# maiziezhoulab/FocalSV

Measured on AMD Instinct MI355X. Metric: target regions/sec (50 kb, 30x HiFi), higher is better.
Workload: dtype u32; 1 GPU; 256 synthetic 50 kb regions per GPU, 30x HiFi-like reads U(10k,20k), 0.2% error, seed 1000+i (BASELINE.json configs[1]); regions_per_gpu=256

## Files before the change

### focalsv_amd/csrc/asm.hip

```cpp
#include "asm_kernels.h"
#include "k_kmer.h"
#include "layout.h"
#include <algorithm>
#include <chrono>
#include <cstdio>
#include <cstdlib>
#include <cstring>
#include <vector>
#include <thread>
#include <atomic>

namespace {

enum { KN_SKETCH, KN_UNIQ, KN_CHAIN, KN_BPM, KN_RESCUE, KN_PATH_FAST, KN_PATH_DP, KN_CONSENSUS, KN_REPACK, KN_EXACT, KN_STITCH, KN_PARTITION, KN_BND, KN_BND_CONS,
       KN_UNIQ_LONG, KN_CHAIN_SPILL,
       KN_COUNT,
       ST_SKETCH = KN_COUNT, ST_CHAIN, ST_VERIFY, ST_PATH, ST_CONSENSUS, ST_FINAL };
const char *const kn_names[KN_COUNT] = {"k_sketch", "k_uniq", "k_chain", "k5_bpm", "k_rescue_accept", "k_path_fast", "k_path_dp", "k_consensus",
                                        "k_repack", "k_exact", "k_stitch", "k_partition", "k_bnd_tasks", "k_bnd_consensus", "k_uniq_long", "k_chain_spill"};
static_assert(KN_COUNT <= FSV_MAX_KERNEL_STATS, "fsv_asm_stats holds every kernel's row");
enum { PASS_NONE = -1, PASS_WINDOWS, PASS_JUNCTIONS, PASS_BCIG, PASS_COUNT };

struct KTimes {
    struct Rec { int k; hipEvent_t a, b; uint64_t bytes; };
// ... 74 lines not shown
    Dev<uint32_t> set_hits;
    Dev<int32_t> len, new_len, idx2, bc_idx;
    Dev<int32_t> bc_win;
    Dev<fsv_mz> mz; Dev<fsv_ovl> ovl, ovl_prev; Dev<fsv_hit> hits, hits_packed; Dev<fsv_piece> pieces; Dev<BndPatch> bnd_patch;
    Dev<fsv_wtask> tasks, tasks2, tasks3; Dev<fsv_wres> res, res2, res3; Dev<fsv_wpath> paths, paths2;
    Dev<uint4> cols_sb, ovl_c, upair_tab, upair_tab_sw, gwin_tab, bc_rec; Dev<uint2> site_rec; Dev<int8_t> site_vec;
    Dev<uint4> uq_ws, spill_list; Dev<uint8_t> spill_slab;
    Dev<uint64_t> cols;
    Dev<unsigned long long> tmp;
    Dev<uint8_t> cov3, bnd_bytes, exact_flag, cwin, thr_tab; Dev<uint16_t> cwin_len; Dev<char> contig_out, contig_all;
    KmerTableState km;
    FilterState fs;
    ChargeState ch;
    std::vector<uint32_t> h_store;
    int occ_sb = 0, occ_fr[3] = {0, 0, 0}, occ_wide = 0;
    ChainArgs last_chain;
    std::vector<uint32_t> h_word_off;
    std::vector<int32_t> h_len;
    const uint32_t *cur_store = nullptr;
    uint32_t n_reads = 0;
    fsv_asm_stats stats;
    uint64_t n_long_reads = 0, n_spilled_pairs = 0;
    KTimes kt;
    void *h_pin = nullptr; size_t h_pin_cap = 0;
    uint32_t *ct_of(int row) { return counters.p + (size_t)row * CT_SLOT; }
    size_t held() const
    {
        return cap_sum(store[0], store[1], cols_sb, contig_all, word_off, len, set_start, read_set, pair_base, mz, mz_off, mz_cnt, ovl, tasks, res, paths,
                       counters, dp_list, dp_list2, dp_list3, dp_list16, dp_list_e3, dp_wide, dp_xwide, cols_wide, set_cols, site_cnt, site_rec, site_off, site_vec,
                       site_cursor, redo, site_lists, read_dirty, cov3, lb, sr_store, brel_off, tasks2, res2, paths2, idx2, bc_idx, bc_rec, bc_win, left_list, fix_list,
// ... 778 lines not shown
    SL.bc_win = W.bc_win.p;
    return FSV_OK;
}

static int consensus_stage(fsv_ctx *ctx, AsmWs &W, Round &R)
{
    const fsv_asm_params &P = R.P; const Batch &B = R.B;
    const uint32_t n_gwin = R.n_gwin;
    TRY(consensus_setup(ctx, W, R));
    const ConsArgs &C = R.C;
    const bool partition = B.n_pairs && P.partition;
    SiteArgs SA{};
    SiteLists SL{};
    if (partition) TRY(partition_setup(ctx, W, R, SA, SL));
    if (partition && P.junction_cigars) TRY(junction_cigars(ctx, W, R, SA, SL));
    const dim3 grid_w((n_gwin + 7u) & ~7u);
    W.kt.begin(ctx, PASS_WINDOWS, KN_CONSENSUS, (uint64_t)n_gwin * (96 + 448));
    if (R.wide_bands) {
        if (partition) FSV_LAUNCH(ctx, ctx->stream, (k_consensus<FSV_EV_CAP_WIDE, 1>), grid_w, dim3(64), 0, C, n_gwin, SL);
        else FSV_LAUNCH(ctx, ctx->stream, (k_consensus<FSV_EV_CAP_WIDE, 0>), grid_w, dim3(64), 0, C, n_gwin, SL);
    } else {
        if (partition) FSV_LAUNCH(ctx, ctx->stream, (k_consensus<FSV_EV_CAP, 1>), grid_w, dim3(64), 0, C, n_gwin, SL);
        else FSV_LAUNCH(ctx, ctx->stream, (k_consensus<FSV_EV_CAP, 0>), grid_w, dim3(64), 0, C, n_gwin, SL);
    }
    W.kt.end(ctx);
    if (partition) {
        const uint32_t grid_l = std::min<uint32_t>(std::max(1u, n_gwin), (uint32_t)ctx->n_cu * 16);
        W.kt.begin(ctx, KN_PARTITION, (uint64_t)B.n_reads * 4);
        FSV_LAUNCH(ctx, ctx->stream, k_snp_sites, dim3(grid_l), dim3(64), 0, C, SA, SL);
        FSV_LAUNCH(ctx, ctx->stream, k_hap_partition, dim3(B.n_reads), dim3(64), 0, C, SA, W.ovl.p, W.ovl_c.p, SL);
// ... 1086 lines not shown
```

### focalsv_amd/csrc/k_consensus.h

```cpp
#pragma once

namespace {

struct ConsArgs {
    const uint32_t *store;
    const uint32_t *word_off;
    const int32_t *read_len;
    const uint32_t *read_set;
    const uint32_t *set_start;
    const uint32_t *pair_base;
    const uint32_t *gwin_off;
    const uint32_t *gwin_read;
    const uint4 *ovl_c;
    const uint4 *gwin_tab;
    const fsv_wtask *tasks;
    const fsv_wpath *paths;
    uint8_t *cwin;
    uint16_t *cwin_len;
    uint32_t *warn;
    uint32_t *changed;
    uint32_t n_reads;
    const uint32_t *read_dirty;
    uint8_t *cov3;
    int junction_vote;
// ... 196 lines not shown
        while (cur >= 0 && cur != S && L < FSV_DG_N) {
            int mx = 0, nx = -1;
            if (L < FSV_INS_MAXLEN + 4) rb[L] = D.base[cur];
            L++;
            for (int i = 0; i < D.in_n[cur]; i++) { const int e = D.in_e[cur][i]; if (D.e_alive[e]) { const int o = D.e_from[e], w = dg_weight(D, o, false); if (w > mx) { mx = w; nx = o; } } }
            cur = nx;
        }
        const int Lc = min(L, FSV_INS_MAXLEN + 4);
        for (int i = 0; i < Lc && i < FSV_INS_MAXLEN; i++) { const uint8_t b = rb[Lc - 1 - i]; seq |= (uint32_t)(b == 'A' ? 0u : b == 'C' ? 1u : b == 'G' ? 2u : 3u) << (2 * i); }
    }
    if (L > FSV_INS_MAXLEN) L = FSV_INS_MAXLEN;
    out_key = ((uint32_t)L << 24) | seq;
    return ws >= we ? ws : we;
}

__device__ __forceinline__ bool poa_decide(const int W[4], const int Ifl[4], int dl, int ni, int mi, uint32_t ikey, int own, bool homo, uint8_t *out)
{
    uint8_t nb = 0;
    bool kept = true;
    for (int visit = 0; visit < 2; visit++) {
        int maxc = -1, type = 0, edge = own, total = 0;
#pragma unroll
        for (int k = 0; k < 4; k++) {
            const int b = k == 0 ? own : (k - 1 < own ? k - 1 : k);
            if (W[b] == 0) continue;
            const int cw = ni ? W[b] - Ifl[b] : W[b];
            total += cw;
            if (cw > maxc) { maxc = cw; type = 0; edge = b; }
        }
        if (ni) { total += ni; if (mi > maxc) { maxc = mi; type = 1; } }
        if (dl) { total += dl; if (dl > maxc) { maxc = dl; type = 2; } }
        if (maxc * 5 >= total * 3 || (homo && maxc * 1000 >= total * 515)) {
            if (type == 1) { const int L = (int)(ikey >> 24); for (int b = 0; b < L; b++) out[1 + nb++] = (uint8_t)((ikey >> (2 * b)) & 3u); ni = 0; continue; }
            if (type == 2) { kept = false; break; }
            out[1 + nb++] = (uint8_t)edge;
            break;
        }
        out[1 + nb++] = (uint8_t)own;
        break;
    }
    out[0] = nb;
    return kept;
}

__device__ __forceinline__ void most_frequent_insertion(const uint32_t *s_evkey, const uint16_t *s_evnext, uint32_t head, int &mi, uint32_t &key)
{
    int bc = 0; uint32_t bk = 0;
    for (uint32_t i = head; i != 0xffffu; i = s_evnext[i]) {
        const uint32_t k1 = s_evkey[i];
        int cn = 0;
        for (uint32_t j2 = head; j2 != 0xffffu; j2 = s_evnext[j2]) cn += (s_evkey[j2] == k1);
        if (cn > bc || (cn == bc && k1 < bk)) { bc = cn; bk = k1; }
    }
    mi = bc; key = bk;
}

#define FSV_INSLIST 128
#define COV_LO(v) ((int)(int16_t)((v) & 0xffff))
#define COV_HI(v) (((int)(v) - COV_LO(v)) >> 16)

template <class F>
__device__ __forceinline__ bool homo_strict(F B, int site, int len)
{
    const int beg = max(0, site - 3), end = min(len - 1, site + 3);
    const uint32_t own = B(site);
    uint32_t f_ch = 4u, b_ch = 4u;
// ... 17 lines not shown
    for (int off = 1; off < 64; off <<= 1) { const int o = __shfl_up(v, off, 64); if (lane >= off) v += o; }
    return v;
}
__device__ __forceinline__ void load_path_ops(const fsv_wpath *P, uint2 (&pv)[13])
{
    const uint2 *src = reinterpret_cast<const uint2 *>(P->ops);
#pragma unroll
    for (int i = 0; i < 13; i++) pv[i] = src[i];
}
__device__ __forceinline__ void lane_columns(int lane, int n, int &c0, int &c1)
{
    const int per = (n + 63) / 64;
    c0 = min(n, lane * per); c1 = min(n, c0 + per);
}

struct TallyCols {
    uint32_t cnt[FSV_WINDOW + 1][3];
    int32_t cov[FSV_WINDOW + 2];
    uint32_t path[64][27];
    uint32_t xraw[28];
    uint32_t cover;

    __device__ __forceinline__ void reset(int lane)
    {
        for (int i = lane; i < (FSV_WINDOW + 1) * 3; i += 64) (&cnt[0][0])[i] = 0;
        for (int i = lane; i < FSV_WINDOW + 2; i += 64) cov[i] = 0;
        if (lane == 0) cover = 0;
    }
    __device__ __forceinline__ void stage_backbone(int lane, const uint32_t *__restrict__ x, int org, int len)
    {
        if (lane < 28) { const int wi = (org >> 4) - 1 + lane; xraw[lane] = (wi >= 0 && wi <= ((len + 15) >> 4)) ? x[wi] : 0u; }
    }
    __device__ __forceinline__ uint32_t xb(int org, int p) const { return (xraw[(p >> 4) - ((org >> 4) - 1)] >> ((p & 15) << 1)) & 3u; }
    __device__ __forceinline__ void cnt_add(int c, uint32_t b) { atomicAdd(&cnt[c][b >> 1], 1u << ((b & 1u) << 4)); }
    __device__ __forceinline__ uint32_t cnt_get(int c, uint32_t b) const { return (cnt[c][b >> 1] >> ((b & 1u) << 4)) & 0xffffu; }
    __device__ __forceinline__ uint32_t stage_path(int lane, const uint2 (&pv)[13])
    {
        uint32_t nz = 0;
#pragma unroll
        for (int i = 0; i < 13; i++) {
            path[lane][2 * i] = pv[i].x; path[lane][2 * i + 1] = pv[i].y;
            nz |= (pv[i].x ? 1u << (2 * i) : 0u) | (pv[i].y ? 2u << (2 * i) : 0u);
        }
        return nz;
    }
};

__device__ __forceinline__ bool split_sub_site(const int oa[4], int occ2, int arrived, int &alt)
{
    const int occ1 = oa[0] + oa[1] + oa[2] + oa[3];
    if (occ1 <= 1) return false;
    const int occ0 = arrived - occ1 - occ2;
    int mx = occ2;
    alt = -1;
#pragma unroll
    for (int b = 0; b < 4; b++) if (oa[b] > mx) { mx = oa[b]; alt = b; }
    if (occ0 == 0 || alt < 0 || mx <= 1) return false;
#pragma unroll
    for (int b = 0; b < 4; b++) if (oa[b] == mx && b != alt) return false;
    return (double)(occ0 + 1 + mx) / (double)(arrived + 1) >= 0.95 && (double)mx / (double)(arrived + 1 - (occ0 + 1)) >= 0.70;
}

template <int EVC>
struct Tally : TallyCols {
    uint32_t evkey[EVC];
    uint32_t evhead[FSV_WINDOW + 1];
    uint32_t fl[FSV_WINDOW + 1];
    uint32_t evn, nins, ndev;
    uint16_t evnext[EVC];
    uint16_t inslist[FSV_INSLIST];
    uint16_t devlist[FSV_WINDOW + 1];
    static_assert(sizeof(DagLds) <= sizeof(uint32_t) * 64 * 27 && (FSV_WINDOW + 1) * 14 <= sizeof(uint32_t) * 64 * 27,
                  "the DAG scratch and the decided columns live in the path buffer between the tally and the write-out");

    __device__ __forceinline__ DagLds &dag() { return *reinterpret_cast<DagLds *>(&path[0][0]); }
    __device__ __forceinline__ uint8_t (*out())[14] { return reinterpret_cast<uint8_t (*)[14]>(&path[0][0]); }

    __device__ __forceinline__ void reset(int lane)
    {
        TallyCols::reset(lane);
        for (int i = lane; i < FSV_WINDOW + 1; i += 64) evhead[i] = 0xffffu;
        for (int i = lane; i < FSV_WINDOW + 1; i += 64) fl[i] = 0;
        if (lane == 0) { evn = 0; nins = 0; ndev = 0; }
    }
    __device__ __forceinline__ void add_event(int c, uint32_t key)
    {
        const uint32_t ev = atomicAdd(&evn, 1u);
        if (ev < (uint32_t)EVC) { evkey[ev] = key; evnext[ev] = (uint16_t)atomicExch(&evhead[c], ev); }
    }

    __device__ __forceinline__ void answer_insertions(int n_cols)
    {
        DagLds &D = dag();
        const int n_list = (int)nins, n = n_list > FSV_INSLIST ? n_cols : n_list;
        for (int li = 0; li < n; li++) {
            const int c = n_list > FSV_INSLIST ? li : (int)inslist[li];
            const uint32_t head = evhead[c] & 0xffffu;
            if (head == 0xffffu || (evhead[c] & 0x10000u)) continue;
            int nk = 0;
            for (uint32_t i = head; i != 0xffffu; i = evnext[i]) { if (nk < FSV_DG_K) D.keys[nk] = evkey[i]; nk++; }
            uint32_t key = 0;
            int mi = dag_insertion(D, nk, key);
            if (mi < 0) most_frequent_insertion(evkey, evnext, head, mi, key);
            evkey[head] = key; evnext[head] = (uint16_t)mi;
            evhead[c] |= 0x10000u;
        }
    }

    template <class F>
    __device__ __forceinline__ bool decide_columns(int lane, int c0, int c1, int org, int n_cols, int len, bool verbatim, int ins_dag, F extra)
    {
        int run = 0, frun = 0;
        for (int c = c0; c < c1; c++) {
            const int v = cov[c];
            run += COV_LO(v); frun += COV_HI(v);
            if (cnt_get(c, 5u)) {
                const uint32_t head = evhead[c];
                bool same = true;
                if (head != 0xffffu) { const uint32_t k0 = evkey[head]; for (uint32_t i = evnext[head]; i != 0xffffu; i = evnext[i]) if (evkey[i] != k0) { same = false; break; } }
                if (!same && ins_dag) { const uint32_t k = atomicAdd(&nins, 1u); if (k < FSV_INSLIST) inslist[k] = (uint16_t)c; }
            }
        }
        int arrived = wave_incl_sum(run, lane) - run, farrived = wave_incl_sum(frun, lane) - frun;
        __syncthreads();
        if (lane == 0 && nins) answer_insertions(n_cols);
        __syncthreads();
        uint8_t (*o)[14] = out();
        for (int c = c0; c < c1; c++) {
            arrived += COV_LO(cov[c]);
            farrived += COV_HI(cov[c]);
            o[c][0] = 1; o[c][1] = (uint8_t)xb(org, org + c);
            if (!verbatim && (cnt[c][0] | cnt[c][1] | cnt[c][2]) != 0u) {
                cov[c] = (int32_t)(((uint32_t)arrived & 0xffffu) | ((uint32_t)farrived << 16));
                devlist[atomicAdd(&ndev, 1u)] = (uint16_t)c;
            }
        }
        __syncthreads();
        bool differs = false;
        for (uint32_t e = lane; e < ndev; e += 64) {
            const int c = (int)devlist[e];
            arrived = (int)(int16_t)((uint32_t)cov[c] & 0xffffu); farrived = (int)(int16_t)((uint32_t)cov[c] >> 16);
            const uint32_t own = xb(org, org + c);
            const bool homo = c > 0 && homo_strict([&](int pp) { return xb(org, pp); }, org + c - 1, len);
            int W[4], Ifl[4], dev = 0;
#pragma unroll
            for (int b = 0; b < 4; b++) { W[b] = (int)cnt_get(c, (uint32_t)b); dev += W[b]; Ifl[b] = (int)((fl[c] >> (b << 3)) & 0xffu); }
            const int dl = (int)cnt_get(c, 4u), ni = (int)cnt_get(c, 5u);
#pragma unroll
            for (int b = 0; b < 4; b++) if ((int)own == b) { W[b] += arrived - dev - dl + 1; Ifl[b] = farrived; }
            int mi = 0; uint32_t ikey = 0;
            if (ni) {
                const uint32_t hv = evhead[c], head = hv & 0xffffu;
                if (head != 0xffffu) {
                    ikey = evkey[head];
                    if (hv & 0x10000u) mi = (int)evnext[head];
                    else if (ins_dag) { for (uint32_t i = head; i != 0xffffu; i = evnext[i]) mi++; }
                    else most_frequent_insertion(evkey, evnext, head, mi, ikey);
                }
            }
            const bool kept = poa_decide(W, Ifl, dl, ni, mi, ikey, (int)own, homo, &o[c][0]);
            extra(c, arrived, kept);
            if (o[c][0] != 1 || o[c][1] != (uint8_t)own) differs = true;
        }
        __syncthreads();
        return differs;
    }
};

#define FSV_PEND_N 4
template <int EVC>
__device__ __forceinline__ void cons_flush(Tally<EVC> &S, const uint32_t *__restrict__ store, uint32_t y_word, int y_len, int y_rev, int ry_start,
                                           const uint32_t (&ent)[FSV_PEND_N], int n)
{
    uint32_t bits[FSV_PEND_N];
#pragma unroll
    for (int i = 0; i < FSV_PEND_N; i++) if (i < n) bits[i] = fetch16(store, y_word, y_len, y_rev, ry_start + (int)((ent[i] >> 9) & 1023u)).bits;
#pragma unroll
// ... 63 lines not shown
    return n2;
}

struct SiteLists {
    uint32_t *site_cnt;
    uint32_t *win_list;
    uint32_t *redo_list;
    uint32_t *win_n;
    const int32_t *bc_win;
};
template <int EVC, int MODE>
__device__ __forceinline__ void consensus_window(const ConsArgs &A, const uint32_t gw, const SiteLists &L)
{
    __shared__ Tally<EVC> S;
    __shared__ uint32_t s_anydev;
    const int lane = threadIdx.x;
    const uint4 gt = A.gwin_tab[gw];
    const uint32_t r = gt.x, pbase = gt.y, n_ovl = gt.z;
    const int g = (int)gt.w;
    const int xlen = A.read_len[r];
    const int gs = g * FSV_WINDOW, glen = min(FSV_WINDOW, xlen - gs);
    S.stage_backbone(lane, A.store + A.word_off[r], gs, xlen);
    uint8_t *dst = A.cwin + (size_t)gw * FSV_CW_STRIDE;
    if (A.read_dirty && !A.read_dirty[r]) {
        __syncthreads();
        for (int c = lane; c < glen; c += 64) dst[c] = (uint8_t)S.xb(gs, gs + c);
        if (lane == 0) { A.cwin_len[gw] = (uint16_t)glen; if (MODE == 1) L.site_cnt[gw] = 0u; }
        return;
    }
    S.reset(lane);
    if (lane == 0) s_anydev = 0;
    __syncthreads();
    for (uint32_t oi = lane; oi < n_ovl; oi += 64) {
        const uint4 oc = A.ovl_c[pbase + oi];
        const int o_x_s = (int)oc.x, o_n_win = (int)(oc.z & 0x7fffffffu);
        const int j = g - o_x_s / FSV_WINDOW;
        if (!(oc.z >> 31) || j < 0 || j >= o_n_win) continue;
        const uint32_t ti = oc.y + (uint32_t)j;
        const fsv_wpath *P = A.paths + ti;
        const uint4 h0 = *reinterpret_cast<const uint4 *>(P);
        const uint2 h1 = *reinterpret_cast<const uint2 *>((const uint8_t *)P + 16);
        uint2 pv[13];
        load_path_ops(P, pv);
        atomicAdd(&S.cover, 1u);
        if ((h0.w & 0xffu) != 1u) continue;
        const bool clean_path = (int16_t)(h0.z >> 16) == 0;
        const uint32_t nz = clean_path ? 0u : S.stage_path(lane, pv);
        const int ry_start = (int)h0.x, plen = (int)(int16_t)(h0.z & 0xffffu);
        const uint32_t y_word = h1.x; const int y_len = (int)h1.y, y_rev = (int)((h0.w >> 8) & 0xffu);
        const int xs = max(gs, o_x_s) - gs;
        bool pend = false;
        if (j > 0 && A.junction_vote) {
            const uint4 hp = *reinterpret_cast<const uint4 *>(A.paths + ti - 1);
            if ((hp.w & 0xffu) == 1u) {
                const int gap = ry_start - (int)hp.y - 1;
                if (gap > 0 && xs == 0) {
                    pend = true;
                    if (gap <= FSV_INS_MAXLEN) {
                        uint32_t key = (uint32_t)gap << 24;
                        for (int b = 0; b < gap; b++) key |= fsv_base_at(A.store, y_word, y_len, y_rev, ry_start - gap + b) << (2 * b);
                        S.add_event(0, key);
                    }
                }
            }
        }
        if (pend || nz) s_anydev = 1u;
        int n2 = 0;
        if (clean_path) { if (pend) S.cnt_add(xs, 5u); }
        else n2 = cons_walk<EVC>(S, S.path[lane], nz, plen, xs, glen, pend, A.store, y_word, y_len, y_rev, ry_start);
        atomicAdd(&S.cov[xs], 1);
        atomicAdd(&S.cov[xs + plen - n2], -1);
    }
    __syncthreads();
    const bool verbatim = S.cover < 3u || s_anydev == 0u;
    if (A.cov3 && lane == 0) A.cov3[gw] = S.cover >= 3u ? 1 : 0;
    if (S.evn > (uint32_t)EVC && lane == 0) atomicOr(&A.warn[r], (uint32_t)FSV_W_INS_EVENTS);
    const int bc_lo = (MODE == 1 && L.bc_win) ? L.bc_win[3 * (size_t)gw + 1] : 1, bc_hi = (MODE == 1 && L.bc_win) ? L.bc_win[3 * (size_t)gw + 2] : 0;
    bool site = false;
    int c0, c1;
    lane_columns(lane, glen, c0, c1);
    const bool differs = S.decide_columns(lane, c0, c1, gs, glen, xlen, verbatim, A.ins_dag, [&](int c, int arrived, bool) {
        if (MODE != 1) return;
        int oa[4], alt;
#pragma unroll
        for (int b = 0; b < 4; b++) oa[b] = (int)S.cnt_get(c, (uint32_t)b);
        if (oa[0] + oa[1] + oa[2] + oa[3] > 1 && c >= bc_lo && c <= bc_hi) site = true;
        if (split_sub_site(oa, (int)S.cnt_get(c, 4u), arrived, alt)) site = true;
    });
    if (differs && A.changed) A.changed[r] = 1u;
    if (MODE == 1) {
        const bool any_site = __ballot(site) != 0ull || (L.bc_win && L.bc_win[3 * (size_t)gw]);
        if (lane == 0) {
            L.site_cnt[gw] = any_site ? FSV_SITE_MARK : 0u;
            if (any_site) L.win_list[atomicAdd(&L.win_n[0], 1u)] = gw;
        }
    }
    uint8_t (*s_out)[14] = S.out();
    uint32_t mine = 0;
    for (int c = c0; c < c1; c++) mine += s_out[c][0];
    const int incl = wave_incl_sum((int)mine, lane);
    uint32_t off = (uint32_t)incl - mine;
    const uint32_t tot = (uint32_t)__shfl(incl, 63, 64);
    if (tot > FSV_CW_STRIDE) {
        for (int c = lane; c < glen; c += 64) dst[c] = (uint8_t)S.xb(gs, gs + c);
        if (lane == 0) { A.cwin_len[gw] = (uint16_t)glen; atomicOr(&A.warn[r], (uint32_t)FSV_W_WINDOW_KEPT); }
        return;
    }
    for (int c = c0; c < c1; c++) for (int b = 0; b < s_out[c][0]; b++) dst[off++] = s_out[c][1 + b];
    if (lane == 0) A.cwin_len[gw] = (uint16_t)tot;
}

template <int EVC, int MODE>
__global__ __launch_bounds__(64) void k_consensus(ConsArgs A, uint32_t n_gwin, SiteLists L)
{
    uint32_t gw;
    if (xcd_block(n_gwin, gw)) consensus_window<EVC, MODE>(A, gw, L);
}

template <int EVC>
__global__ __launch_bounds__(64) void k_consensus_redo(ConsArgs A, SiteLists L)
{
    const uint32_t n = L.win_n[1];
    for (uint32_t i = blockIdx.x; i < n; i += gridDim.x) {
// ... 175 lines not shown
    uint32_t *site_cnt;
    uint2 *site_rec;
    uint32_t *site_off;
    uint32_t *rec_cursor; uint32_t rec_cap;
    int8_t *vec;
    uint32_t *vec_cursor;
    uint32_t vec_cap;
    uint32_t *read_sites;
    const int32_t *bc_idx;
    const uint4 *bc_rec;
    const fsv_wpath *bc_paths;
};

__device__ __forceinline__ void snp_sites_window(const ConsArgs &A, const uint32_t gw, const SiteArgs &S)
{
    __shared__ TallyCols T;
    __shared__ uint8_t s_alt[FSV_WINDOW + 1];
    __shared__ uint8_t s_sidx[FSV_WINDOW + 1];
    __shared__ uint32_t s_nsite, s_vbase, s_rbase;
    __shared__ uint32_t s_scan[64];
    const int lane = threadIdx.x;
    const uint4 gt = A.gwin_tab[gw];
    const uint32_t r = gt.x, pbase = gt.y, n_ovl = gt.z;
    const int g = (int)gt.w;
    const int xlen = A.read_len[r];
    const int gs = g * FSV_WINDOW, glen = min(FSV_WINDOW, xlen - gs);
    if (lane == 0) S.site_cnt[gw] = 0;
    T.stage_backbone(lane, A.store + A.word_off[r], gs, xlen);
    T.reset(lane);
    for (int i = lane; i < FSV_WINDOW + 1; i += 64) s_alt[i] = 0;
    if (lane == 0) s_nsite = 0;
// ... 378 lines not shown
                                                     const uint32_t *__restrict__ n3)
{
    const uint32_t j = blockIdx.x * blockDim.x + threadIdx.x;
    if (j < *n3) res2[src3[j]] = res3[j];
}

struct BndPatch { uint16_t ts, told, tnew, hs, hold, hnew, valid, pad; };

template <int EVC>
__global__ __launch_bounds__(64) void k_bnd_consensus(ConsArgs A, BndArgs B, const fsv_wpath *__restrict__ paths2, const uint32_t *__restrict__ store2,
                                                      BndPatch *__restrict__ patch, uint8_t *__restrict__ patch_bytes)
{
    static_assert(2 * FSV_BND_HALF + 1 <= FSV_WINDOW, "a junction's backbone fits the tally of a window");
    struct Lds : Tally<EVC> {
        uint32_t terr;
        uint16_t off[FSV_WINDOW + 2];
        uint8_t own[FSV_WINDOW + 1];
    };
    __shared__ Lds S;
    const int lane = threadIdx.x;
    const uint32_t n_list = *B.n_bnd;
    for (uint32_t li = blockIdx.x; li < n_list; li += gridDim.x) {
        __syncthreads();
        const uint32_t gw = B.bnd_list[li];
        const uint4 gt = A.gwin_tab[gw];
        const uint32_t r = gt.x, pbase = gt.y, n_ovl = gt.z;
        const int g = (int)gt.w;
        const int gs = g * FSV_WINDOW;
        const int LB = (int)B.lb[gw], len_now = LB + (int)B.cwin_len[gw];
        const int cws = max(0, LB - FSV_BND_HALF), cwe = min(len_now - 1, LB + FSV_BND_HALF - 1), blen = cwe - cws + 1;
        if (lane == 0) { patch[gw].valid = 0; S.terr = 0; }
        S.stage_backbone(lane, store2 + B.b_base + B.brel_off[r], cws, len_now);
        S.reset(lane);
        __syncthreads();
        for (uint32_t oi = lane; oi < n_ovl; oi += 64) {
            const uint4 oc = A.ovl_c[pbase + oi];
            const int o_x_s = (int)oc.x, o_n_win = (int)(oc.z & 0x7fffffffu);
            const int j = g - o_x_s / FSV_WINDOW;
            if (!(oc.z >> 31) || j < 0 || j >= o_n_win || o_x_s > gs) continue;
            const int32_t slot = B.idx2[oc.y + (uint32_t)j];
            if (slot == -2) { atomicAdd(&S.cover, 1u); atomicAdd(&S.cov[0], 1); atomicAdd(&S.cov[blen], -1); continue; }
            if (slot < 0) continue;
            const fsv_wpath *P = paths2 + slot;
            const uint4 h0 = *reinterpret_cast<const uint4 *>(P);
            if ((h0.w & 0xffu) != 1u) continue;
            const uint2 h1 = *reinterpret_cast<const uint2 *>((const uint8_t *)P + 16);
            const int perr = (int)(int16_t)(h0.z >> 16);
            atomicAdd(&S.cover, 1u);
            const int ry_start = (int)h0.x, plen = (int)(int16_t)(h0.z & 0xffffu);
            int n2 = 0;
            if (perr != 0) {
                atomicAdd(&S.terr, (uint32_t)perr);
                uint2 pv[13];
                load_path_ops(P, pv);
                const uint32_t nz = S.stage_path(lane, pv);
                n2 = cons_walk<EVC>(S, S.path[lane], nz, plen, 0, blen, false, A.store, h1.x, (int)h1.y, (int)((h0.w >> 8) & 0xffu), ry_start);
            }
            atomicAdd(&S.cov[0], 1);
            atomicAdd(&S.cov[plen - n2], -1);
        }
        __syncthreads();
        if (S.cover < 3u || S.terr == 0u) continue;
        if (S.evn > (uint32_t)EVC && lane == 0) atomicOr(&A.warn[r], (uint32_t)FSV_W_INS_EVENTS);
        int c0, c1;
        lane_columns(lane, blen, c0, c1);
        for (int c = c0; c < c1; c++) S.own[c] = 1;
        const bool differs = S.decide_columns(lane, c0, c1, cws, blen, len_now, false, A.ins_dag, [&](int c, int, bool kept) { S.own[c] = kept; });
        uint8_t (*s_out)[14] = S.out();
        int mine = 0;
        for (int c = c0; c < c1; c++) mine += s_out[c][0];
        if (__ballot(differs) == 0ull) continue;
        int off = wave_incl_sum(mine, lane) - mine;
        for (int c = c0; c < c1; c++) { S.off[c] = (uint16_t)off; off += s_out[c][0]; }
        const int sb = FSV_BND_SIDE, eb = blen - 1 - FSV_BND_SIDE;
        int fs = 0x7fffffff, fe = 0x7fffffff;
        for (int c = c0; c < c1; c++) { if (S.own[c] && c >= sb && c < fs) fs = c; if (S.own[c] && c >= eb && c < fe) fe = c; }
        for (int d = 32; d >= 1; d >>= 1) { fs = min(fs, __shfl_xor(fs, d)); fe = min(fe, __shfl_xor(fe, d)); }
        __syncthreads();
        if (eb <= sb || fs == 0x7fffffff || fe == 0x7fffffff) continue;
        const int o0 = (int)S.off[fs] + s_out[fs][0] - 1, o1 = (int)S.off[fe] + s_out[fe][0] - 1;
        const int R0 = cws + fs, R1 = cws + fe, sc = LB - cws;
        const int o_split = sc <= fs ? o0 : (sc > fe ? o1 + 1 : (int)S.off[sc]);
        const int lb_prev = (int)B.lb[gw - 1];
        BndPatch bp;
        bp.valid = 1; bp.pad = 0;
        bp.ts = (uint16_t)max(0, R0 - lb_prev); bp.told = (uint16_t)max(0, min(R1, LB - 1) - R0 + 1); bp.tnew = (uint16_t)(o_split - o0);
        bp.hs = (uint16_t)(max(R0, LB) - LB); bp.hold = (uint16_t)max(0, R1 - max(R0, LB) + 1); bp.hnew = (uint16_t)(o1 + 1 - o_split);
        if (R0 < lb_prev || o1 + 1 - o0 > FSV_CW_STRIDE) {
            if (lane == 0) atomicOr(&A.warn[r], (uint32_t)FSV_W_WINDOW_KEPT);
            continue;
        }
        uint8_t *dst = patch_bytes + (size_t)gw * FSV_CW_STRIDE;
        for (int c = c0; c < c1; c++)
            for (int b = 0; b < s_out[c][0]; b++) { const int pos = (int)S.off[c] + b; if (pos >= o0 && pos <= o1) dst[pos - o0] = s_out[c][1 + b]; }
        if (lane == 0) patch[gw] = bp;
    }
}

__global__ __launch_bounds__(64) void k_bnd_apply(const uint32_t *__restrict__ gwin_read, const uint32_t *__restrict__ gwin_off, const BndPatch *__restrict__ patch,
                                                  const uint8_t *__restrict__ patch_bytes, const uint32_t *__restrict__ bnd_flag, uint32_t n_gwin,
                                                  uint8_t *__restrict__ cwin, uint16_t *__restrict__ cwin_len, uint32_t *__restrict__ changed, uint32_t *__restrict__ warn)
{
    __shared__ uint8_t s_old[FSV_CW_STRIDE];
    const uint32_t gw = blockIdx.x;
    if (gw >= n_gwin) return;
    const uint32_t r = gwin_read[gw];
    const bool has_h = gw > gwin_off[r] && (bnd_flag[gw] & 1u) && patch[gw].valid;
    const bool has_t = gw + 1 < gwin_off[r + 1] && (bnd_flag[gw + 1] & 1u) && patch[gw + 1].valid;
    if (!has_h && !has_t) return;
// ... 30 lines not shown
```

Measured before the change: 2529 regions/s.

## Shrink consensus LDS footprint to fit more windows per CU

Cuts the consensus and junction-consensus tally shared memory. The per-lane path staging shrinks from 64 rows to 31 rows, processed in ballot-ranked batches. Decided columns are packed into one byte each, with insertion bases re-read from the event key at write-out, and event heads become 16-bit packed words updated by CAS. The goal is to raise resident blocks per CU (a static_assert targets 12) so memory and atomic latency is hidden better. The cost is extra loop passes and syncthreads when more than 31 lanes need path walks, plus CAS loops on the event heads.

```diff
diff --git a/focalsv_amd/csrc/asm.hip b/focalsv_amd/csrc/asm.hip
--- a/focalsv_amd/csrc/asm.hip
+++ b/focalsv_amd/csrc/asm.hip
@@ -112,6 +112,7 @@
     ChargeState ch;
     std::vector<uint32_t> h_store;
     int occ_sb = 0, occ_fr[3] = {0, 0, 0}, occ_wide = 0;
+    int occ_cons = 0;
     ChainArgs last_chain;
     std::vector<uint32_t> h_word_off;
     std::vector<int32_t> h_len;
@@ -920,6 +921,12 @@
     SiteLists SL{};
     if (partition) TRY(partition_setup(ctx, W, R, SA, SL));
     if (partition && P.junction_cigars) TRY(junction_cigars(ctx, W, R, SA, SL));
+    if (!W.occ_cons) {
+        FSV_HIP(ctx, hipOccupancyMaxActiveBlocksPerMultiprocessor(&W.occ_cons, (k_consensus<FSV_EV_CAP, 1>), 64, 0));
+        int occ_bnd = 0;
+        FSV_HIP(ctx, hipOccupancyMaxActiveBlocksPerMultiprocessor(&occ_bnd, k_bnd_consensus<FSV_EV_CAP>, 64, 0));
+        if (getenv("FSV_TRACE")) fprintf(stderr, "[fsv] asm blocks per CU: k_consensus %d, k_bnd_consensus %d\n", W.occ_cons, occ_bnd);
+    }
     const dim3 grid_w((n_gwin + 7u) & ~7u);
     W.kt.begin(ctx, PASS_WINDOWS, KN_CONSENSUS, (uint64_t)n_gwin * (96 + 448));
     if (R.wide_bands) {
diff --git a/focalsv_amd/csrc/k_consensus.h b/focalsv_amd/csrc/k_consensus.h
--- a/focalsv_amd/csrc/k_consensus.h
+++ b/focalsv_amd/csrc/k_consensus.h
@@ -234,9 +234,14 @@
     return ws >= we ? ws : we;
 }
 
-__device__ __forceinline__ bool poa_decide(const int W[4], const int Ifl[4], int dl, int ni, int mi, uint32_t ikey, int own, bool homo, uint8_t *out)
-{
-    uint8_t nb = 0;
+#define FSV_OUT_NB(o) ((o) & 15u)
+#define FSV_OUT_BASE(o) (((o) >> 4) & 3u)
+#define FSV_OUT_INS 0x40u
+#define FSV_OUT_KEPT 0x80u
+static_assert(FSV_INS_MAXLEN + 1 <= 15, "the bases written for a column are counted in four bits");
+__device__ __forceinline__ uint32_t poa_decide(const int W[4], const int Ifl[4], int dl, int ni, int mi, uint32_t ikey, int own, bool homo)
+{
+    uint32_t nb = 0, ins = 0, fin = (uint32_t)own;
     bool kept = true;
     for (int visit = 0; visit < 2; visit++) {
         int maxc = -1, type = 0, edge = own, total = 0;
@@ -251,25 +256,26 @@
         if (ni) { total += ni; if (mi > maxc) { maxc = mi; type = 1; } }
         if (dl) { total += dl; if (dl > maxc) { maxc = dl; type = 2; } }
         if (maxc * 5 >= total * 3 || (homo && maxc * 1000 >= total * 515)) {
-            if (type == 1) { const int L = (int)(ikey >> 24); for (int b = 0; b < L; b++) out[1 + nb++] = (uint8_t)((ikey >> (2 * b)) & 3u); ni = 0; continue; }
+            if (type == 1) { nb += ikey >> 24; ins = FSV_OUT_INS; ni = 0; continue; }
             if (type == 2) { kept = false; break; }
-            out[1 + nb++] = (uint8_t)edge;
+            nb++; fin = (uint32_t)edge;
             break;
         }
-        out[1 + nb++] = (uint8_t)own;
+        nb++;
         break;
     }
-    out[0] = nb;
-    return kept;
-}
-
+    return nb | (fin << 4) | ins | (kept ? FSV_OUT_KEPT : 0u);
+}
+
+#define FSV_EV_END 0x7fffu
+#define FSV_EV_ANSWERED 0x8000u
 __device__ __forceinline__ void most_frequent_insertion(const uint32_t *s_evkey, const uint16_t *s_evnext, uint32_t head, int &mi, uint32_t &key)
 {
     int bc = 0; uint32_t bk = 0;
-    for (uint32_t i = head; i != 0xffffu; i = s_evnext[i]) {
+    for (uint32_t i = head; i != FSV_EV_END; i = s_evnext[i]) {
         const uint32_t k1 = s_evkey[i];
         int cn = 0;
-        for (uint32_t j2 = head; j2 != 0xffffu; j2 = s_evnext[j2]) cn += (s_evkey[j2] == k1);
+        for (uint32_t j2 = head; j2 != FSV_EV_END; j2 = s_evnext[j2]) cn += (s_evkey[j2] == k1);
         if (cn > bc || (cn == bc && k1 < bk)) { bc = cn; bk = k1; }
     }
     mi = bc; key = bk;
@@ -317,10 +323,13 @@
     c0 = min(n, lane * per); c1 = min(n, c0 + per);
 }
 
+#define FSV_TALLY_ROWS 31
+#define FSV_TALLY_LDS_MAX 13648
+template <int ROWS>
 struct TallyCols {
     uint32_t cnt[FSV_WINDOW + 1][3];
     int32_t cov[FSV_WINDOW + 2];
-    uint32_t path[64][27];
+    uint32_t path[ROWS][27];
     uint32_t xraw[28];
     uint32_t cover;
 
@@ -337,12 +346,12 @@
     __device__ __forceinline__ uint32_t xb(int org, int p) const { return (xraw[(p >> 4) - ((org >> 4) - 1)] >> ((p & 15) << 1)) & 3u; }
     __device__ __forceinline__ void cnt_add(int c, uint32_t b) { atomicAdd(&cnt[c][b >> 1], 1u << ((b & 1u) << 4)); }
     __device__ __forceinline__ uint32_t cnt_get(int c, uint32_t b) const { return (cnt[c][b >> 1] >> ((b & 1u) << 4)) & 0xffffu; }
-    __device__ __forceinline__ uint32_t stage_path(int lane, const uint2 (&pv)[13])
+    __device__ __forceinline__ uint32_t stage_path(int row, const uint2 (&pv)[13])
     {
         uint32_t nz = 0;
 #pragma unroll
         for (int i = 0; i < 13; i++) {
-            path[lane][2 * i] = pv[i].x; path[lane][2 * i + 1] = pv[i].y;
+            path[row][2 * i] = pv[i].x; path[row][2 * i + 1] = pv[i].y;
             nz |= (pv[i].x ? 1u << (2 * i) : 0u) | (pv[i].y ? 2u << (2 * i) : 0u);
         }
         return nz;
@@ -364,49 +373,81 @@
     return (double)(occ0 + 1 + mx) / (double)(arrived + 1) >= 0.95 && (double)mx / (double)(arrived + 1 - (occ0 + 1)) >= 0.70;
 }
 
+struct tally_rows {
+    int n_need, rank; bool need;
+    __device__ __forceinline__ tally_rows(bool need_, int lane) : need(need_)
+    {
+        const uint64_t m = __ballot(need_);
+        n_need = __popcll(m); rank = __popcll(m & ((1ull << lane) - 1ull));
+    }
+    __device__ __forceinline__ bool mine(int first) const { return need && rank >= first && rank < first + FSV_TALLY_ROWS; }
+};
+
 template <int EVC>
-struct Tally : TallyCols {
+struct Tally : TallyCols<FSV_TALLY_ROWS> {
+    using Cols = TallyCols<FSV_TALLY_ROWS>;
     uint32_t evkey[EVC];
-    uint32_t evhead[FSV_WINDOW + 1];
+    uint32_t evhead2[(FSV_WINDOW + 2) / 2];
     uint32_t fl[FSV_WINDOW + 1];
     uint32_t evn, nins, ndev;
     uint16_t evnext[EVC];
     uint16_t inslist[FSV_INSLIST];
-    uint16_t devlist[FSV_WINDOW + 1];
-    static_assert(sizeof(DagLds) <= sizeof(uint32_t) * 64 * 27 && (FSV_WINDOW + 1) * 14 <= sizeof(uint32_t) * 64 * 27,
-                  "the DAG scratch and the decided columns live in the path buffer between the tally and the write-out");
-
-    __device__ __forceinline__ DagLds &dag() { return *reinterpret_cast<DagLds *>(&path[0][0]); }
-    __device__ __forceinline__ uint8_t (*out())[14] { return reinterpret_cast<uint8_t (*)[14]>(&path[0][0]); }
+    static_assert(EVC <= (int)FSV_EV_END, "an event index fits the 15 bits of a list head");
+    static constexpr int WORK_OUT = 0, WORK_DEV = WORK_OUT + ((FSV_WINDOW + 1 + 3) & ~3), WORK_OFF = WORK_DEV + (((FSV_WINDOW + 1) * 2 + 3) & ~3),
+                         WORK_END = WORK_OFF + (FSV_WINDOW + 2) * 2;
+    static_assert(sizeof(DagLds) <= sizeof(uint32_t) * FSV_TALLY_ROWS * 27 && WORK_END <= (int)(sizeof(uint32_t) * FSV_TALLY_ROWS * 27),
+                  "the DAG scratch, then the decided columns with the deviation list and the offsets, live in the path rows after the tally");
+
+    __device__ __forceinline__ uint8_t *work() { return reinterpret_cast<uint8_t *>(&path[0][0]); }
+    __device__ __forceinline__ DagLds &dag() { return *reinterpret_cast<DagLds *>(work()); }
+    __device__ __forceinline__ uint8_t *out() { return work() + WORK_OUT; }
+    __device__ __forceinline__ uint16_t *devlist() { return reinterpret_cast<uint16_t *>(work() + WORK_DEV); }
+    __device__ __forceinline__ uint16_t *col_off() { return reinterpret_cast<uint16_t *>(work() + WORK_OFF); }
+    __device__ __forceinline__ uint16_t *heads() { return reinterpret_cast<uint16_t *>(evhead2); }
+    template <class F>
+    __device__ __forceinline__ void emit_column(int c, F put)
+    {
+        const uint32_t o = out()[c], nb = FSV_OUT_NB(o);
+        if (!(o & FSV_OUT_INS)) { if (nb) put((uint8_t)FSV_OUT_BASE(o)); return; }
+        const uint32_t key = evkey[heads()[c] & FSV_EV_END], L = key >> 24;
+        for (uint32_t b = 0; b < nb; b++) put((uint8_t)(b < L ? (key >> (2u * b)) & 3u : FSV_OUT_BASE(o)));
+    }
 
     __device__ __forceinline__ void reset(int lane)
     {
-        TallyCols::reset(lane);
-        for (int i = lane; i < FSV_WINDOW + 1; i += 64) evhead[i] = 0xffffu;
+        Cols::reset(lane);
+        for (int i = lane; i < (FSV_WINDOW + 2) / 2; i += 64) evhead2[i] = FSV_EV_END | (FSV_EV_END << 16);
         for (int i = lane; i < FSV_WINDOW + 1; i += 64) fl[i] = 0;
         if (lane == 0) { evn = 0; nins = 0; ndev = 0; }
     }
     __device__ __forceinline__ void add_event(int c, uint32_t key)
     {
         const uint32_t ev = atomicAdd(&evn, 1u);
-        if (ev < (uint32_t)EVC) { evkey[ev] = key; evnext[ev] = (uint16_t)atomicExch(&evhead[c], ev); }
+        if (ev >= (uint32_t)EVC) return;
+        evkey[ev] = key;
+        uint32_t *w = &evhead2[c >> 1];
+        const uint32_t sh = (uint32_t)(c & 1) << 4;
+        uint32_t seen = *w, was;
+        do { was = seen; seen = atomicCAS(w, was, (was & ~(0xffffu << sh)) | (ev << sh)); } while (seen != was);
+        evnext[ev] = (uint16_t)((was >> sh) & 0xffffu);
     }
 
     __device__ __forceinline__ void answer_insertions(int n_cols)
     {
         DagLds &D = dag();
+        uint16_t *evhead = heads();
         const int n_list = (int)nins, n = n_list > FSV_INSLIST ? n_cols : n_list;
         for (int li = 0; li < n; li++) {
             const int c = n_list > FSV_INSLIST ? li : (int)inslist[li];
-            const uint32_t head = evhead[c] & 0xffffu;
-            if (head == 0xffffu || (evhead[c] & 0x10000u)) continue;
+            const uint32_t head = evhead[c] & FSV_EV_END;
+            if (head == FSV_EV_END || (evhead[c] & FSV_EV_ANSWERED)) continue;
             int nk = 0;
-            for (uint32_t i = head; i != 0xffffu; i = evnext[i]) { if (nk < FSV_DG_K) D.keys[nk] = evkey[i]; nk++; }
+            for (uint32_t i = head; i != FSV_EV_END; i = evnext[i]) { if (nk < FSV_DG_K) D.keys[nk] = evkey[i]; nk++; }
             uint32_t key = 0;
             int mi = dag_insertion(D, nk, key);
             if (mi < 0) most_frequent_insertion(evkey, evnext, head, mi, key);
             evkey[head] = key; evnext[head] = (uint16_t)mi;
-            evhead[c] |= 0x10000u;
+            evhead[c] = (uint16_t)(head | FSV_EV_ANSWERED);
         }
     }
 
@@ -418,9 +459,9 @@
             const int v = cov[c];
             run += COV_LO(v); frun += COV_HI(v);
             if (cnt_get(c, 5u)) {
-                const uint32_t head = evhead[c];
+                const uint32_t head = heads()[c];
                 bool same = true;
-                if (head != 0xffffu) { const uint32_t k0 = evkey[head]; for (uint32_t i = evnext[head]; i != 0xffffu; i = evnext[i]) if (evkey[i] != k0) { same = false; break; } }
+                if (head != FSV_EV_END) { const uint32_t k0 = evkey[head]; for (uint32_t i = evnext[head]; i != FSV_EV_END; i = evnext[i]) if (evkey[i] != k0) { same = false; break; } }
                 if (!same && ins_dag) { const uint32_t k = atomicAdd(&nins, 1u); if (k < FSV_INSLIST) inslist[k] = (uint16_t)c; }
             }
         }
@@ -428,20 +469,21 @@
         __syncthreads();
         if (lane == 0 && nins) answer_insertions(n_cols);
         __syncthreads();
-        uint8_t (*o)[14] = out();
+        uint8_t *o = out();
+        uint16_t *dl_cols = devlist();
         for (int c = c0; c < c1; c++) {
             arrived += COV_LO(cov[c]);
             farrived += COV_HI(cov[c]);
-            o[c][0] = 1; o[c][1] = (uint8_t)xb(org, org + c);
+            o[c] = (uint8_t)(1u | (xb(org, org + c) << 4) | FSV_OUT_KEPT);
             if (!verbatim && (cnt[c][0] | cnt[c][1] | cnt[c][2]) != 0u) {
                 cov[c] = (int32_t)(((uint32_t)arrived & 0xffffu) | ((uint32_t)farrived << 16));
-                devlist[atomicAdd(&ndev, 1u)] = (uint16_t)c;
+                dl_cols[atomicAdd(&ndev, 1u)] = (uint16_t)c;
             }
         }
         __syncthreads();
         bool differs = false;
         for (uint32_t e = lane; e < ndev; e += 64) {
-            const int c = (int)devlist[e];
+            const int c = (int)dl_cols[e];
             arrived = (int)(int16_t)((uint32_t)cov[c] & 0xffffu); farrived = (int)(int16_t)((uint32_t)cov[c] >> 16);
             const uint32_t own = xb(org, org + c);
             const bool homo = c > 0 && homo_strict([&](int pp) { return xb(org, pp); }, org + c - 1, len);
@@ -453,17 +495,19 @@
             for (int b = 0; b < 4; b++) if ((int)own == b) { W[b] += arrived - dev - dl + 1; Ifl[b] = farrived; }
             int mi = 0; uint32_t ikey = 0;
             if (ni) {
-                const uint32_t hv = evhead[c], head = hv & 0xffffu;
-                if (head != 0xffffu) {
+                const uint32_t hv = heads()[c], head = hv & FSV_EV_END;
+                if (head != FSV_EV_END) {
                     ikey = evkey[head];
-                    if (hv & 0x10000u) mi = (int)evnext[head];
-                    else if (ins_dag) { for (uint32_t i = head; i != 0xffffu; i = evnext[i]) mi++; }
-                    else most_frequent_insertion(evkey, evnext, head, mi, ikey);
+                    if (hv & FSV_EV_ANSWERED) mi = (int)evnext[head];
+                    else if (ins_dag) { for (uint32_t i = head; i != FSV_EV_END; i = evnext[i]) mi++; }
+                    else { most_frequent_insertion(evkey, evnext, head, mi, ikey); evkey[head] = ikey; }
                 }
             }
-            const bool kept = poa_decide(W, Ifl, dl, ni, mi, ikey, (int)own, homo, &o[c][0]);
-            extra(c, arrived, kept);
-            if (o[c][0] != 1 || o[c][1] != (uint8_t)own) differs = true;
+            const uint32_t d = poa_decide(W, Ifl, dl, ni, mi, ikey, (int)own, homo);
+            o[c] = (uint8_t)d;
+            extra(c, arrived, (d & FSV_OUT_KEPT) != 0u);
+            const uint32_t first = ((d & FSV_OUT_INS) && (ikey >> 24)) ? (ikey & 3u) : FSV_OUT_BASE(d);
+            if (FSV_OUT_NB(d) != 1u || first != own) differs = true;
         }
         __syncthreads();
         return differs;
@@ -557,6 +601,7 @@
 {
     __shared__ Tally<EVC> S;
     __shared__ uint32_t s_anydev;
+    static_assert(EVC != FSV_EV_CAP || sizeof(Tally<EVC>) + sizeof(uint32_t) <= FSV_TALLY_LDS_MAX, "k_consensus / k_consensus_redo: 12 windows per CU");
     const int lane = threadIdx.x;
     const uint4 gt = A.gwin_tab[gw];
     const uint32_t r = gt.x, pbase = gt.y, n_ovl = gt.z;
@@ -574,45 +619,66 @@
     S.reset(lane);
     if (lane == 0) s_anydev = 0;
     __syncthreads();
-    for (uint32_t oi = lane; oi < n_ovl; oi += 64) {
-        const uint4 oc = A.ovl_c[pbase + oi];
-        const int o_x_s = (int)oc.x, o_n_win = (int)(oc.z & 0x7fffffffu);
-        const int j = g - o_x_s / FSV_WINDOW;
-        if (!(oc.z >> 31) || j < 0 || j >= o_n_win) continue;
-        const uint32_t ti = oc.y + (uint32_t)j;
-        const fsv_wpath *P = A.paths + ti;
-        const uint4 h0 = *reinterpret_cast<const uint4 *>(P);
-        const uint2 h1 = *reinterpret_cast<const uint2 *>((const uint8_t *)P + 16);
+    for (uint32_t ob = 0; ob < n_ovl; ob += 64) {
+        const uint32_t oi = ob + lane;
+        bool live = false, walks = false, pend = false;
+        const fsv_wpath *P = nullptr;
+        int ry_start = 0, plen = 0, y_len = 0, y_rev = 0, xs = 0;
+        uint32_t y_word = 0;
         uint2 pv[13];
-        load_path_ops(P, pv);
-        atomicAdd(&S.cover, 1u);
-        if ((h0.w & 0xffu) != 1u) continue;
-        const bool clean_path = (int16_t)(h0.z >> 16) == 0;
-        const uint32_t nz = clean_path ? 0u : S.stage_path(lane, pv);
-        const int ry_start = (int)h0.x, plen = (int)(int16_t)(h0.z & 0xffffu);
-        const uint32_t y_word = h1.x; const int y_len = (int)h1.y, y_rev = (int)((h0.w >> 8) & 0xffu);
-        const int xs = max(gs, o_x_s) - gs;
-        bool pend = false;
-        if (j > 0 && A.junction_vote) {
-            const uint4 hp = *reinterpret_cast<const uint4 *>(A.paths + ti - 1);
-            if ((hp.w & 0xffu) == 1u) {
-                const int gap = ry_start - (int)hp.y - 1;
-                if (gap > 0 && xs == 0) {
-                    pend = true;
-                    if (gap <= FSV_INS_MAXLEN) {
-                        uint32_t key = (uint32_t)gap << 24;
-                        for (int b = 0; b < gap; b++) key |= fsv_base_at(A.store, y_word, y_len, y_rev, ry_start - gap + b) << (2 * b);
-                        S.add_event(0, key);
+        if (oi < n_ovl) {
+            const uint4 oc = A.ovl_c[pbase + oi];
+            const int o_x_s = (int)oc.x, o_n_win = (int)(oc.z & 0x7fffffffu);
+            const int j = g - o_x_s / FSV_WINDOW;
+            if ((oc.z >> 31) && j >= 0 && j < o_n_win) {
+                const uint32_t ti = oc.y + (uint32_t)j;
+                P = A.paths + ti;
+                const uint4 h0 = *reinterpret_cast<const uint4 *>(P);
+                const uint2 h1 = *reinterpret_cast<const uint2 *>((const uint8_t *)P + 16);
+                load_path_ops(P, pv);
+                atomicAdd(&S.cover, 1u);
+                if ((h0.w & 0xffu) == 1u) {
+                    live = true;
+                    walks = (int16_t)(h0.z >> 16) != 0;
+                    ry_start = (int)h0.x; plen = (int)(int16_t)(h0.z & 0xffffu);
+                    y_word = h1.x; y_len = (int)h1.y; y_rev = (int)((h0.w >> 8) & 0xffu);
+                    xs = max(gs, o_x_s) - gs;
+                    if (j > 0 && A.junction_vote) {
+                        const uint4 hp = *reinterpret_cast<const uint4 *>(A.paths + ti - 1);
+                        if ((hp.w & 0xffu) == 1u) {
+                            const int gap = ry_start - (int)hp.y - 1;
+                            if (gap > 0 && xs == 0) {
+                                pend = true;
+                                if (gap <= FSV_INS_MAXLEN) {
+                                    uint32_t key = (uint32_t)gap << 24;
+                                    for (int b = 0; b < gap; b++) key |= fsv_base_at(A.store, y_word, y_len, y_rev, ry_start - gap + b) << (2 * b);
+                                    S.add_event(0, key);
+                                }
+                            }
+                        }
                     }
+                    if (pend) s_anydev = 1u;
                 }
             }
         }
-        if (pend || nz) s_anydev = 1u;
+        const tally_rows rows(walks, lane);
+        uint32_t nz = 0;
+        if (rows.mine(0)) nz = S.stage_path(rows.rank, pv);
         int n2 = 0;
-        if (clean_path) { if (pend) S.cnt_add(xs, 5u); }
-        else n2 = cons_walk<EVC>(S, S.path[lane], nz, plen, xs, glen, pend, A.store, y_word, y_len, y_rev, ry_start);
-        atomicAdd(&S.cov[xs], 1);
-        atomicAdd(&S.cov[xs + plen - n2], -1);
+        for (int first = 0; first < rows.n_need; first += FSV_TALLY_ROWS) {
+            if (rows.mine(first)) {
+                const int row = rows.rank - first;
+                if (first) { uint2 pw[13]; load_path_ops(P, pw); nz = S.stage_path(row, pw); }
+                if (nz) s_anydev = 1u;
+                n2 = cons_walk<EVC>(S, S.path[row], nz, plen, xs, glen, pend, A.store, y_word, y_len, y_rev, ry_start);
+            }
+            __syncthreads();
+        }
+        if (live) {
+            if (!walks && pend) S.cnt_add(xs, 5u);
+            atomicAdd(&S.cov[xs], 1);
+            atomicAdd(&S.cov[xs + plen - n2], -1);
+        }
     }
     __syncthreads();
     const bool verbatim = S.cover < 3u || s_anydev == 0u;
@@ -638,9 +704,9 @@
             if (any_site) L.win_list[atomicAdd(&L.win_n[0], 1u)] = gw;
         }
     }
-    uint8_t (*s_out)[14] = S.out();
+    const uint8_t *s_out = S.out();
     uint32_t mine = 0;
-    for (int c = c0; c < c1; c++) mine += s_out[c][0];
+    for (int c = c0; c < c1; c++) mine += FSV_OUT_NB(s_out[c]);
     const int incl = wave_incl_sum((int)mine, lane);
     uint32_t off = (uint32_t)incl - mine;
     const uint32_t tot = (uint32_t)__shfl(incl, 63, 64);
@@ -649,7 +715,7 @@
         if (lane == 0) { A.cwin_len[gw] = (uint16_t)glen; atomicOr(&A.warn[r], (uint32_t)FSV_W_WINDOW_KEPT); }
         return;
     }
-    for (int c = c0; c < c1; c++) for (int b = 0; b < s_out[c][0]; b++) dst[off++] = s_out[c][1 + b];
+    for (int c = c0; c < c1; c++) S.emit_column(c, [&](uint8_t b) { dst[off++] = b; });
     if (lane == 0) A.cwin_len[gw] = (uint16_t)tot;
 }
 
@@ -855,7 +921,7 @@
 
 __device__ __forceinline__ void snp_sites_window(const ConsArgs &A, const uint32_t gw, const SiteArgs &S)
 {
-    __shared__ TallyCols T;
+    __shared__ TallyCols<64> T;
     __shared__ uint8_t s_alt[FSV_WINDOW + 1];
     __shared__ uint8_t s_sidx[FSV_WINDOW + 1];
     __shared__ uint32_t s_nsite, s_vbase, s_rbase;
@@ -1264,10 +1330,9 @@
     static_assert(2 * FSV_BND_HALF + 1 <= FSV_WINDOW, "a junction's backbone fits the tally of a window");
     struct Lds : Tally<EVC> {
         uint32_t terr;
-        uint16_t off[FSV_WINDOW + 2];
-        uint8_t own[FSV_WINDOW + 1];
     };
     __shared__ Lds S;
+    static_assert(EVC != FSV_EV_CAP || sizeof(Lds) <= FSV_TALLY_LDS_MAX, "k_bnd_consensus: 12 junctions per CU");
     const int lane = threadIdx.x;
     const uint32_t n_list = *B.n_bnd;
     for (uint32_t li = blockIdx.x; li < n_list; li += gridDim.x) {
@@ -1283,54 +1348,73 @@
         S.stage_backbone(lane, store2 + B.b_base + B.brel_off[r], cws, len_now);
         S.reset(lane);
         __syncthreads();
-        for (uint32_t oi = lane; oi < n_ovl; oi += 64) {
-            const uint4 oc = A.ovl_c[pbase + oi];
-            const int o_x_s = (int)oc.x, o_n_win = (int)(oc.z & 0x7fffffffu);
-            const int j = g - o_x_s / FSV_WINDOW;
-            if (!(oc.z >> 31) || j < 0 || j >= o_n_win || o_x_s > gs) continue;
-            const int32_t slot = B.idx2[oc.y + (uint32_t)j];
-            if (slot == -2) { atomicAdd(&S.cover, 1u); atomicAdd(&S.cov[0], 1); atomicAdd(&S.cov[blen], -1); continue; }
-            if (slot < 0) continue;
-            const fsv_wpath *P = paths2 + slot;
-            const uint4 h0 = *reinterpret_cast<const uint4 *>(P);
-            if ((h0.w & 0xffu) != 1u) continue;
-            const uint2 h1 = *reinterpret_cast<const uint2 *>((const uint8_t *)P + 16);
-            const int perr = (int)(int16_t)(h0.z >> 16);
-            atomicAdd(&S.cover, 1u);
-            const int ry_start = (int)h0.x, plen = (int)(int16_t)(h0.z & 0xffffu);
+        for (uint32_t ob = 0; ob < n_ovl; ob += 64) {
+            const uint32_t oi = ob + lane;
+            bool live = false, walks = false;
+            const fsv_wpath *P = nullptr;
+            int ry_start = 0, plen = 0, y_len = 0, y_rev = 0;
+            uint32_t y_word = 0;
+            if (oi < n_ovl) {
+                const uint4 oc = A.ovl_c[pbase + oi];
+                const int o_x_s = (int)oc.x, o_n_win = (int)(oc.z & 0x7fffffffu);
+                const int j = g - o_x_s / FSV_WINDOW;
+                if ((oc.z >> 31) && j >= 0 && j < o_n_win && o_x_s <= gs) {
+                    const int32_t slot = B.idx2[oc.y + (uint32_t)j];
+                    if (slot == -2) { atomicAdd(&S.cover, 1u); atomicAdd(&S.cov[0], 1); atomicAdd(&S.cov[blen], -1); }
+                    else if (slot >= 0) {
+                        P = paths2 + slot;
+                        const uint4 h0 = *reinterpret_cast<const uint4 *>(P);
+                        if ((h0.w & 0xffu) == 1u) {
+                            const uint2 h1 = *reinterpret_cast<const uint2 *>((const uint8_t *)P + 16);
+                            const int perr = (int)(int16_t)(h0.z >> 16);
+                            atomicAdd(&S.cover, 1u);
+                            live = true; walks = perr != 0;
+                            ry_start = (int)h0.x; plen = (int)(int16_t)(h0.z & 0xffffu);
+                            y_word = h1.x; y_len = (int)h1.y; y_rev = (int)((h0.w >> 8) & 0xffu);
+                            if (walks) atomicAdd(&S.terr, (uint32_t)perr);
+                        }
+                    }
+                }
+            }
+            const tally_rows rows(walks, lane);
             int n2 = 0;
-            if (perr != 0) {
-                atomicAdd(&S.terr, (uint32_t)perr);
-                uint2 pv[13];
-                load_path_ops(P, pv);
-                const uint32_t nz = S.stage_path(lane, pv);
-                n2 = cons_walk<EVC>(S, S.path[lane], nz, plen, 0, blen, false, A.store, h1.x, (int)h1.y, (int)((h0.w >> 8) & 0xffu), ry_start);
-            }
-            atomicAdd(&S.cov[0], 1);
-            atomicAdd(&S.cov[plen - n2], -1);
+            for (int first = 0; first < rows.n_need; first += FSV_TALLY_ROWS) {
+                if (rows.mine(first)) {
+                    const int row = rows.rank - first;
+                    uint2 pv[13];
+                    load_path_ops(P, pv);
+                    const uint32_t nz = S.stage_path(row, pv);
+                    n2 = cons_walk<EVC>(S, S.path[row], nz, plen, 0, blen, false, A.store, y_word, y_len, y_rev, ry_start);
+                }
+                __syncthreads();
+            }
+            if (live) {
+                atomicAdd(&S.cov[0], 1);
+                atomicAdd(&S.cov[plen - n2], -1);
+            }
         }
         __syncthreads();
         if (S.cover < 3u || S.terr == 0u) continue;
         if (S.evn > (uint32_t)EVC && lane == 0) atomicOr(&A.warn[r], (uint32_t)FSV_W_INS_EVENTS);
         int c0, c1;
         lane_columns(lane, blen, c0, c1);
-        for (int c = c0; c < c1; c++) S.own[c] = 1;
-        const bool differs = S.decide_columns(lane, c0, c1, cws, blen, len_now, false, A.ins_dag, [&](int c, int, bool kept) { S.own[c] = kept; });
-        uint8_t (*s_out)[14] = S.out();
+        const bool differs = S.decide_columns(lane, c0, c1, cws, blen, len_now, false, A.ins_dag, [](int, int, bool) {});
+        const uint8_t *s_out = S.out();
+        uint16_t *s_off = S.col_off();
         int mine = 0;
-        for (int c = c0; c < c1; c++) mine += s_out[c][0];
+        for (int c = c0; c < c1; c++) mine += (int)FSV_OUT_NB(s_out[c]);
         if (__ballot(differs) == 0ull) continue;
         int off = wave_incl_sum(mine, lane) - mine;
-        for (int c = c0; c < c1; c++) { S.off[c] = (uint16_t)off; off += s_out[c][0]; }
+        for (int c = c0; c < c1; c++) { s_off[c] = (uint16_t)off; off += (int)FSV_OUT_NB(s_out[c]); }
         const int sb = FSV_BND_SIDE, eb = blen - 1 - FSV_BND_SIDE;
         int fs = 0x7fffffff, fe = 0x7fffffff;
-        for (int c = c0; c < c1; c++) { if (S.own[c] && c >= sb && c < fs) fs = c; if (S.own[c] && c >= eb && c < fe) fe = c; }
+        for (int c = c0; c < c1; c++) { const bool own = (s_out[c] & FSV_OUT_KEPT) != 0u; if (own && c >= sb && c < fs) fs = c; if (own && c >= eb && c < fe) fe = c; }
         for (int d = 32; d >= 1; d >>= 1) { fs = min(fs, __shfl_xor(fs, d)); fe = min(fe, __shfl_xor(fe, d)); }
         __syncthreads();
         if (eb <= sb || fs == 0x7fffffff || fe == 0x7fffffff) continue;
-        const int o0 = (int)S.off[fs] + s_out[fs][0] - 1, o1 = (int)S.off[fe] + s_out[fe][0] - 1;
+        const int o0 = (int)s_off[fs] + (int)FSV_OUT_NB(s_out[fs]) - 1, o1 = (int)s_off[fe] + (int)FSV_OUT_NB(s_out[fe]) - 1;
         const int R0 = cws + fs, R1 = cws + fe, sc = LB - cws;
-        const int o_split = sc <= fs ? o0 : (sc > fe ? o1 + 1 : (int)S.off[sc]);
+        const int o_split = sc <= fs ? o0 : (sc > fe ? o1 + 1 : (int)s_off[sc]);
         const int lb_prev = (int)B.lb[gw - 1];
         BndPatch bp;
         bp.valid = 1; bp.pad = 0;
@@ -1341,8 +1425,10 @@
             continue;
         }
         uint8_t *dst = patch_bytes + (size_t)gw * FSV_CW_STRIDE;
-        for (int c = c0; c < c1; c++)
-            for (int b = 0; b < s_out[c][0]; b++) { const int pos = (int)S.off[c] + b; if (pos >= o0 && pos <= o1) dst[pos - o0] = s_out[c][1 + b]; }
+        for (int c = c0; c < c1; c++) {
+            int pos = (int)s_off[c];
+            S.emit_column(c, [&](uint8_t b) { if (pos >= o0 && pos <= o1) dst[pos - o0] = b; pos++; });
+        }
         if (lane == 0) patch[gw] = bp;
     }
 }
```

Measured after the change: 2692 regions/s, median of 4. +6.5%, better.
